# dlavado/scene-net

Measured on AMD Instinct MI355X. Metric: voxel-tiles/sec (point cloud -> 64^3 occupancy -> 16-GENEO bank conv -> head), higher is better.
Workload: dtype i8; 1 GPU; C2: 32 tiles/GPU x 100000 points (fp64 xyz, UTM-scale), 64^3 voxel grid, 16 GENEO kernels 9^3 (cy 6, cone 5, neg 5); conv on the int8 matrix cores: binary occupancy x 24-bit fixed-point weights (3 int8 digits), exact int32 accumulation, fp32 head; tiles_per_gpu=32, points_per_tile=100000, geneo_kernels=16, parallelism=tile-sharded x1, no collectives

## Files before the change

include/scenenet_hip.h:

```cpp
#ifndef SCENENET_HIP_H
#define SCENENET_HIP_H

#include <stddef.h>
#include <stdint.h>

#ifdef __cplusplus
extern "C" {
#endif

typedef void* sn_stream_t;

typedef enum {
    SN_OK = 0,
    SN_ERR_INVALID_ARG = -1,
    SN_ERR_UNSUPPORTED = -2,
    SN_ERR_LAUNCH = -3,
    SN_ERR_NO_DEVICE = -4,
    SN_ERR_DEVICE_STATUS = -5
} sn_status;

typedef enum { SN_F32 = 0, SN_F64 = 1, SN_U8 = 2, SN_OCC8 = 3, SN_BF16 = 4, SN_I32 = 5 } sn_dtype;

typedef enum {
    SN_GENEO_CY = 0, SN_GENEO_CONE = 1, SN_GENEO_NEG = 2,
// ... 38 lines not shown
                 void* act, void* out, int out_dtype, sn_stream_t stream);

int sn_conv_bank_plan(int x_dtype, int B, int Z, int X, int Y, int G, int kz, int kx, int ky, int32_t* plan8);

#define SN_CONV_PREP_BYTES 16384
int sn_conv_bank_prep(const float* bank, int G, int kz, int kx, int ky, void* prep, sn_stream_t stream);
int sn_conv_bank_prepared(const void* x, int x_dtype, const float* bank, const float* lambdas, void* prep,
                          int B, int Z, int X, int Y, int G, int kz, int kx, int ky,
                          void* act, void* out, int out_dtype, sn_stream_t stream);
int sn_conv_bank_prepared_served(const void* x, int x_dtype, const float* bank, const float* lambdas, void* prep,
                                 int B, int Z, int X, int Y, int G, int kz, int kx, int ky,
                                 void* act, void* out, int out_dtype, sn_stream_t stream);
int sn_conv_prep_verdict_offset(void);
int sn_conv_i8_spin_timeouts(unsigned long long* count);
int sn_conv_i8z_round_counts(unsigned long long* counts2);
int sn_voxel_onepass_giveups(unsigned long long* count);

int sn_launch_timing_events(void* start_event, void* stop_event);

int sn_conv_fused(const void* x, int x_dtype, const float* bank, const float* lambdas, int B, int Z, int X, int Y,
                  int G, int kz, int kx, int ky, void* out, int out_dtype, sn_stream_t stream);
int sn_conv_fused_v(const void* x, int x_dtype, const float* bank, const float* lambdas, int B, int Z, int X, int Y, int G,
                    int kz, int kx, int ky, void* out, int out_dtype, int32_t* verdict, int assume_served,
                    sn_stream_t stream);
size_t sn_conv_fused_prep_bytes(int kz, int kx, int ky);
int sn_conv_fused_prep(const float* bank, const float* lambdas, int G, int kz, int kx, int ky, void* blob,
                       sn_stream_t stream);
int sn_conv_fused_prepared(const void* x, int x_dtype, const float* bank, const float* lambdas, const void* blob, int B,
                           int Z, int X, int Y, int G, int kz, int kx, int ky, void* out, int out_dtype, int assume_served,
                           sn_stream_t stream);
// ... 406 lines not shown
```

scene-net_amd/_hip.py:

```python
from __future__ import annotations

import contextlib
import ctypes
import functools
import os
from ctypes import c_char_p, c_int, c_void_p
from typing import NamedTuple, Optional, Sequence, Tuple

import torch

_HERE = os.path.dirname(os.path.abspath(__file__))
LIB_PATH = os.environ.get("SN_HIP_LIB") or os.path.join(_HERE, "lib", "libscenenet_hip.so")

SN_F32, SN_F64, SN_U8, SN_OCC8, SN_BF16, SN_I32 = 0, 1, 2, 3, 4, 5
SN_GENEO_CY, SN_GENEO_CONE, SN_GENEO_NEG = 0, 1, 2
SN_GENEO_CY_V1, SN_GENEO_CONE_V1, SN_GENEO_NEG_V1 = 3, 4, 5
SN_P_RADIUS, SN_P_SIGMA, SN_P_APEX, SN_P_CONE_RADIUS, SN_P_CONE_INC, SN_P_NEG_FACTOR = 0, 1, 2, 3, 4, 5
SN_NPARAM = 8

_P, _I = c_void_p, c_int
SYMBOLS = {
    "sn_version": (c_int, []),
    "sn_prepare_device": (c_int, []),
    "sn_device_status": (c_int, [_P, _P]),
# ... 2 lines not shown
    "sn_device_count": (c_int, []),
    "sn_conv_i8_path_counts": (c_int, [_P]),
    "sn_set_option": (c_int, [c_char_p, _I]),
    "sn_get_option": (c_int, [c_char_p]),
    "sn_geneo_bank": (c_int, [_P, _P, _I, _I, _I, _I, _P, _P, _P]),
    "sn_effective_lambdas": (c_int, [_P, _P, _I, _I, _P, _P]),
    "sn_conv_bank": (c_int, [_P, _I, _P, _P, _I, _I, _I, _I, _I, _I, _I, _I, _P, _P, _I, _P]),
    "sn_conv_bank_plan": (c_int, [_I, _I, _I, _I, _I, _I, _I, _I, _I, _P]),
    "sn_geneo_bank_prep": (c_int, [_P, _P, _I, _I, _I, _I, _P, _P, _P, _P, _I, _P, _P, _P]),
    "sn_conv_bank_prep": (c_int, [_P, _I, _I, _I, _I, _P, _P]),
    "sn_conv_bank_prepared": (c_int, [_P, _I, _P, _P, _P, _I, _I, _I, _I, _I, _I, _I, _I, _P, _P, _I, _P]),
    "sn_conv_bank_prepared_served": (c_int, [_P, _I, _P, _P, _P, _I, _I, _I, _I, _I, _I, _I, _I, _P, _P, _I, _P]),
    "sn_conv_prep_verdict_offset": (c_int, []),
    "sn_conv_i8_spin_timeouts": (c_int, [_P]),
    "sn_conv_i8z_round_counts": (c_int, [_P]),
    "sn_voxel_onepass_giveups": (c_int, [_P]),
    "sn_launch_timing_events": (c_int, [_P, _P]),
    "sn_conv_fused": (c_int, [_P, _I, _P, _P, _I, _I, _I, _I, _I, _I, _I, _I, _P, _I, _P]),
    "sn_conv_fused_supported": (c_int, [_I, _I, _I, _I, _I, _I, _I]),
    "sn_forward_auto": (c_int, [_P, _I, _P, _P, _I, _I, _I, _I, _I, _I, _I, _I, _P, _P, _P, _I, _P]),
    "sn_voxel_bbox": (c_int, [_P, _P, _I, _P, _P]),
    "sn_voxel_desc": (c_int, [_P, _I, _I, _I, _I, _I, _P, _P]),
    "sn_voxel_desc_from_bounds": (c_int, [_P, _I, _I, _I, _I, _P, _P]),
    "sn_voxel_desc_sized": (c_int, [_P, _I, _P, _I, _I, _I, _P, _P, _P, _P]),
    "sn_voxel_finalize_sized": (c_int, [_P, _P, _I, _I, _I, _I, _P, _P, _P, _P, _P, _P, _P]),
    "sn_voxel_scatter": (c_int, [_P, _P, _P, _I, _P, _I, _I, _I, _P, _P, _P, _I, _P, _P]),
    "sn_voxel_finalize": (c_int, [_P, _P, _I, _I, _I, _I, _P, _P, _P, _P, _P, _P]),
    "sn_voxel_occupancy": (c_int, [_P, _P, _P, _I, _P, _I, _I, _I, _P, _I, _P, _P, _P, _I, _P, _P, _P, _P, _P]),
    "sn_voxel_occupancy_fused": (c_int, [_P, _P, _P, _I, _I, _I, _I, _I, _P, _I, _P, _P, _P, _P, _P, _P, _I, _P, _P, _P, _P,
                                         _P]),
# ... 209 lines not shown
    return int(buf[0]), int(buf[1]), int(buf[2])


def conv_i8_spin_timeouts() -> int:
    buf = (ctypes.c_ulonglong * 1)()
    _check(load().sn_conv_i8_spin_timeouts(ctypes.cast(buf, ctypes.c_void_p)), "sn_conv_i8_spin_timeouts")
    return int(buf[0])


def conv_i8z_round_counts() -> Tuple[int, int]:
    buf = (ctypes.c_ulonglong * 2)()
    _check(load().sn_conv_i8z_round_counts(ctypes.cast(buf, ctypes.c_void_p)), "sn_conv_i8z_round_counts")
    return int(buf[0]), int(buf[1])


def voxel_onepass_giveups() -> int:
    buf = (ctypes.c_ulonglong * 1)()
    _check(load().sn_voxel_onepass_giveups(ctypes.cast(buf, ctypes.c_void_p)), "sn_voxel_onepass_giveups")
    return int(buf[0])


def launch_timing_events(start: "torch.cuda.Event", stop: "torch.cuda.Event") -> None:
    a, b = int(start.cuda_event), int(stop.cuda_event)
    if not a or not b:
        raise HipLibraryError("launch_timing_events: record each event once first (torch creates the handle lazily)")
    _check_plain(load().sn_launch_timing_events(ctypes.c_void_p(a), ctypes.c_void_p(b)), "sn_launch_timing_events")


def _ptr(t: Optional[torch.Tensor], dtype: Optional[torch.dtype] = None, name: str = "tensor") -> Optional[int]:
    if t is None:
# ... 1728 lines not shown
```

scene-net_amd/csrc/cabi.hip:

```cpp
#include "common.h"
#include <climits>
#include <cstdlib>
#include <cstring>

#include <atomic>
#include <mutex>
#include <unordered_map>

namespace sn {
char* error_buffer() {
    static thread_local char buf[512] = {0};
    return buf;
}
namespace {
struct Option {
    const char* name;
    const char* env;
    int on;
    int def, lo, hi;
    bool is_switch;
    std::atomic<int> value{env ? -1 : def};
};
Option g_options[] = {
    {"conv_skip_empty_tiles",  nullptr,                 0,  0,       0,  1,       true},
    {"conv_i8_tolerance_ppb",  nullptr,                 0,  90000,   0,  INT_MAX, false},
    {"conv_i8_fold",           "SN_CONV_I8_NOFOLD",     0,  1,       0,  1,       true},
    {"conv_i8_legacy",         "SN_CONV_I8_LEGACY",     1,  0,       0,  1,       true},
    {"conv_i8_no_stage",       "SN_CONV_I8_NO_STAGE",   1,  0,       0,  1,       true},
    {"conv_i8z_variant",       nullptr,                 0,  2,       0,  2,       false},
    {"conv_no_i8",             "SN_CONV_NO_I8",         1,  0,       0,  1,       true},
    {"conv_double_buffer",     "SN_CONV_DOUBLE_BUFFER", 1,  0,       0,  1,       true},
    {"conv_lin_no24",          "SN_CONV_LIN_NO24",      1,  0,       0,  1,       true},
    {"voxel_onepass",          nullptr,                 0,  1,       0,  1,       true},
    {"voxel_onepass_spin",     nullptr,                 0,  64,      0,  INT_MAX, false},
    {"corr_dense",             "SN_CORR_DENSE",         1,  0,       0,  1,       true},
    {"corr_sparse_tile_bytes", nullptr,                 0,  0,       0,  2048,    false},
    {"conv_i8z_inject_fault",  nullptr,                 0,  0,       0,  1,       true},
    {"conv_i8z_segments",      nullptr,                 0,  0,       0,  4,       false},
    {"conv_i8z_dense",         nullptr,                 0,  0,       0,  1,       true},
};
static_assert(sizeof(g_options) / sizeof(g_options[0]) == kOptCount, "one entry per sn::Opt");
}

int option(Opt which) {
    Option& o = g_options[which];
    int v = o.value.load(std::memory_order_relaxed);
    if (v < 0) {
        const char* e = getenv(o.env);
        int expected = -1;
        o.value.compare_exchange_strong(expected, (e && e[0] == '1') ? o.on : o.def, std::memory_order_relaxed);
        v = o.value.load(std::memory_order_relaxed);
    }
    return v;
// ... 194 lines not shown
```

scene-net_amd/csrc/common.h:

```cpp
#pragma once
#include <hip/hip_runtime.h>
#include <cstdarg>
#include <cstdio>
#include <cstdlib>
#include "scenenet_hip.h"

namespace sn {

char* error_buffer();

inline int fail(int code, const char* fmt, ...) {
    va_list ap;
    va_start(ap, fmt);
    vsnprintf(error_buffer(), 512, fmt, ap);
    va_end(ap);
    return code;
}

int sticky_check(const char* what);

inline int check_launch(const char* what) {
    hipError_t e = hipGetLastError();
    if (e != hipSuccess) return fail(SN_ERR_LAUNCH, "%s: %s", what, hipGetErrorString(e));
    return sticky_check(what);
// ... 5 lines not shown
    kOptConvSkipEmptyTiles,
    kOptConvI8TolerancePpb,
    kOptConvI8Fold,
    kOptConvI8Legacy,
    kOptConvI8NoStage,
    kOptConvI8zVariant,
    kOptConvNoI8,
    kOptConvDoubleBuffer,
    kOptConvLinNo24,
    kOptVoxelOnepass,
    kOptVoxelOnepassSpin,
    kOptCorrDense,
    kOptCorrSparseTileBytes,
    kOptConvI8zInjectFault,
    kOptConvI8zSegments,
    kOptConvI8zDense,
    kOptCount
};
int option(Opt which);
inline float conv_i8_tolerance() { return 1e-9f * (float)option(kOptConvI8TolerancePpb); }

hipError_t ensure_dynamic_lds(const void* kernel, int bytes);

constexpr int kGateDepth = 3;
struct Gate {
    const int32_t* ptr[kGateDepth];
    int want[kGateDepth];
    __device__ __forceinline__ bool pass() const {
#pragma unroll
        for (int i = 0; i < kGateDepth; ++i)
// ... 67 lines not shown
```

scene-net_amd/csrc/conv_i8s.hip:

```cpp
#include "common.h"
#include <hip/hip_ext.h>
#include <cstdlib>
#include <cstring>
#include <type_traits>
#include <vector>

namespace {

#include "conv_prep.h"
#include "conv_fp32.inc"

#include "conv_i8_common.inc"
#include "conv_i8s_kernel.inc"
#include "conv_i8f.inc"

size_t lds_bytes_fold(const Shape& s) {
    const size_t hdw = (size_t)s.ZP * s.XP * DW;
    const size_t ring = kNB * hdw * 4, alias = 2 * hdw * 4 + ((size_t)s.G * 729 + 1) * sizeof(float);
    return (size_t)kFoldSteps * 3 * 64 * 16 + 64 + 64 + 128 + 128 + 64 + sizeof(FoldPlan) +
           (ring > alias ? ring : alias) + 16;
}

void plan_fold(int XP, FoldPlan& p) {
    for (int qq = 0; qq < 4; ++qq) {
// ... 244 lines not shown
    }
    if (best_cost < 0) return 1;
    if (!z.dense && SN_I8Z_SKIP_NSEG > 0 && SN_I8Z_SKIP_NSEG <= max_seg &&
        (ncol * SN_I8Z_SKIP_NSEG + cus - 1) / cus <= kZMaxJobs) {
        best_seg = SN_I8Z_SKIP_NSEG;
        z.deal = 1;
        z.deal_shift = SN_I8Z_SKIP_SHIFT;
    } else if (!z.dense) {
        const int want = sn::option(sn::kOptConvI8zSegments);
        const int n = want >= 2 ? want : (want == 0 && !act && z.nxt >= 2 && Z >= 32 && best_seg == 1) ? 2 : 0;
        if (n >= 2 && n <= max_seg && (ncol * n + cus - 1) / cus <= kZMaxJobs) {
            best_seg = n;
            z.deal = 1;
            z.deal_shift = z.nxt / n > 1 ? z.nxt / n : 1;
            z.fill_dead = act ? 0 : 1;
        }
    }
    z.LZ = (Z + best_seg - 1) / best_seg;
    z.nseg = (Z + z.LZ - 1) / z.LZ;
    z.PL = z.LZ + 8;
    const long long njobs = ncol * z.nseg;
    if (njobs > 0x7fffffff) return 1;
    z.njobs = (int)njobs;
    const int grid = (int)(njobs < cus ? njobs : cus);
    const int per_wg = (z.njobs + grid - 1) / grid;
    if (per_wg > kZMaxJobs) return 1;
    if (!division_magic((unsigned)z.PL, (unsigned)(per_wg * z.PL + 64), z.pl_magic)) return 1;
    z.swizzle = (grid % 8 == 0) ? 1 : 0;
    const size_t lds = lds_bytes_zwalk();
    const size_t lds_4 = lds_bytes(s4), lds_f = fp32k::lds_bytes(cs, false);
    const size_t lds_fb = lds_4 > lds_f ? lds_4 : lds_f;
    if (lds > (size_t)kMaxLds || lds_fb > (size_t)kMaxLds) return 1;
    hipEvent_t t_start = nullptr, t_stop = nullptr;
    sn::take_timing_events(t_start, t_stop);
#define SN_LAUNCH_I8Z(OT, KH, KR, KW)                                                                            \
    do {                                                                                                         \
        auto kern = act ? conv_occ_i8z_kernel<OT, KH, KR, KW, true> : conv_occ_i8z_kernel<OT, KH, KR, KW, false>; \
        if (sn::ensure_dynamic_lds((const void*)kern, kMaxLds) != hipSuccess)                                    \
            return check_launch("sn_conv_bank_prepared(i8z: hipFuncSetAttribute)");                              \
        if (t_start || t_stop)               \
            hipExtLaunchKernelGGL(kern, dim3(grid), dim3(64 * KW), (uint32_t)lds, stream, t_start, t_stop, 0u, x, lambdas,  \
                                  (const uint8_t*)prep, z, (OT*)act, (OT*)out);                                   \
        else                                                                                                     \
            hipLaunchKernelGGL(kern, dim3(grid), dim3(64 * KW), lds, stream, x, lambdas, (const uint8_t*)prep, z,   \
// ... 98 lines not shown
                                            void* out, int out_dtype, sn_stream_t stream) {
    return conv_bank_prepared_impl(x, x_dtype, bank, lambdas, prep, B, Z, X, Y, G, kz, kx, ky, act, out, out_dtype, stream, 1);
}

extern "C" int sn_conv_prep_verdict_offset(void) { return kPrepRoute; }

extern "C" int sn_conv_i8_path_counts(unsigned long long* counts3) {
    if (!counts3) return sn::fail(SN_ERR_INVALID_ARG, "sn_conv_i8_path_counts: null pointer");
    unsigned long long h[4] = {0, 0, 0, 0};
    if (hipDeviceSynchronize() != hipSuccess || hipMemcpyFromSymbol(h, HIP_SYMBOL(g_fold_counts), sizeof(h)) != hipSuccess)
        return sn::check_launch("sn_conv_i8_path_counts");
    counts3[0] = h[0]; counts3[1] = h[1]; counts3[2] = h[2];
    return SN_OK;
}

extern "C" int sn_conv_i8z_round_counts(unsigned long long* counts2) {
    if (!counts2) return sn::fail(SN_ERR_INVALID_ARG, "sn_conv_i8z_round_counts: null pointer");
    unsigned long long h[2] = {0, 0};
    if (hipDeviceSynchronize() != hipSuccess || hipMemcpyFromSymbol(h, HIP_SYMBOL(g_zwalk_rounds), sizeof(h)) != hipSuccess)
        return sn::check_launch("sn_conv_i8z_round_counts");
    counts2[0] = h[0]; counts2[1] = h[1];
    return SN_OK;
}

extern "C" int sn_conv_i8_spin_timeouts(unsigned long long* count) {
    if (!count) return sn::fail(SN_ERR_INVALID_ARG, "sn_conv_i8_spin_timeouts: null pointer");
    unsigned long long h[4] = {0, 0, 0, 0};
    if (hipDeviceSynchronize() != hipSuccess || hipMemcpyFromSymbol(h, HIP_SYMBOL(g_fold_counts), sizeof(h)) != hipSuccess)
        return sn::check_launch("sn_conv_i8_spin_timeouts");
    *count = h[3];
// ... 11 lines not shown
```

scene-net_amd/csrc/conv_i8z.inc:

```

constexpr int kZTX = 8;
constexpr int kZRows = kZTX + 8;
constexpr int kZRing = 16;
#ifndef SN_I8Z_LAG
#define SN_I8Z_LAG 3
#endif
constexpr int kZLag = SN_I8Z_LAG;
constexpr int kZD = 8 + kZLag;
#ifndef SN_I8Z_DD
#define SN_I8Z_DD 4
#endif
constexpr int kZDD = SN_I8Z_DD;
constexpr int kZPre = kZD + kZDD;
constexpr int kZRawPlane = kZRows * DW * 4;
constexpr int kZYqRow = 256, kZYqPlane = kZRows * kZYqRow;
constexpr int kZYcRow = 64, kZYcPlane = kZRows * kZYcRow + 32;
constexpr int kZMaxJobs = 256;
#ifndef SN_I8Z_SKIP_NSEG
#define SN_I8Z_SKIP_NSEG 0
#endif
#ifndef SN_I8Z_SKIP_SHIFT
#define SN_I8Z_SKIP_SHIFT 0
#endif
#ifndef SN_I8Z_AHEAD
// ... 14 lines not shown
    int njobs;
    unsigned pl_magic;
    int swizzle;
    float tol;
    sn::Gate gate;
    int32_t* route;
    int served;
    int fill_dead;
    int32_t* sticky;
    int dbg;
    int dense;
    int deal, deal_shift;
};

__device__ unsigned long long g_zwalk_rounds[2] = {0ull, 0ull};

__device__ __forceinline__ int zjob_id(const ZShape& z, int wg, int k, int grid) {
    const int base = k * grid;
    if (z.swizzle && base + grid <= z.njobs) return base + (wg & 7) * (grid >> 3) + (wg >> 3);
    return base + wg;
}

constexpr int kPrepThreads = SN_BANK_THREADS;
__global__ __launch_bounds__(kPrepThreads) void conv_prep_kernel(const float* __restrict__ bank, int G,
                                                                 uint8_t* __restrict__ prep) {
    __shared__ __align__(16) float w[732 + kPrepScratchWords];
    const int g = blockIdx.x, tid = threadIdx.x;
    const bool valid = g < G;
    for (int i = tid; i < 729; i += kPrepThreads) w[i] = valid ? bank[(size_t)g * 729 + i] : 0.0f;
    prep_one_kernel(w, w + 732, valid, g, prep, tid, kPrepThreads);
// ... 189 lines not shown
    const int lane = tid & 63, wave = __builtin_amdgcn_readfirstlane(tid >> 6);
    uint4* Wd = reinterpret_cast<uint4*>(lds);
    int4* jobtab = reinterpret_cast<int4*>(Wd + kFoldSteps * 3 * 64);
    float* scale = reinterpret_cast<float*>(jobtab + kZMaxJobs);
    float* lamsc = scale + 16;
    float* lamhi = lamsc + 16;
    double* bnd = reinterpret_cast<double*>(lamhi + 32);
    int* cnt = reinterpret_cast<int*>(bnd + 16);
    int4* chk = reinterpret_cast<int4*>(cnt + 128);
    int4* ltab = chk + 64;
    int4* stab = ltab + 64;
    uint32_t* rowmask = reinterpret_cast<uint32_t*>(stab + 64);
    uint8_t* raw = reinterpret_cast<uint8_t*>(rowmask + 32);
    uint8_t* Yc = raw + kZRing * kZRawPlane;
    uint8_t* Yq = Yc + kZRing * kZYcPlane;
    int* const ticket_ctr = cnt + 96;

#ifdef SN_CONV_TIMING
    if (lane < 8 && wave < 8) g_i8s_w[(blockIdx.x * 8 + wave) * 8 + lane] = 0;
#define SN_ZT(k, t0) do { if (lane == 0 && wave < 8) g_i8s_w[(blockIdx.x * 8 + wave) * 8 + (k)] += clock64() - (t0); } while (0)
#define SN_ZNOW() clock64()
#else
#define SN_ZT(k, t0) do { (void)(t0); } while (0)
#define SN_ZNOW() 0ull
#endif
    SN_ST(0);
    const size_t V = (size_t)zs.Z * zs.X * zs.Y;
    const int grid = (int)gridDim.x;
    const int dealt = (int)blockIdx.x < zs.njobs ? (zs.njobs - 1 - (int)blockIdx.x) / grid + 1 : 0;
    int my_jobs = dealt;
    int NPL = my_jobs * zs.PL;
    int nslots = NPL + kZD;
    const bool fill_dead = kLean && zs.fill_dead != 0;
    int* const live = reinterpret_cast<int*>(Yq);
    if (tid < 128) cnt[tid] = 0;
    if (tid >= 128 && tid < 192) {
        const int l = tid - 128, i = l & 15, role = l >> 4;
        int4 e = make_int4(0, 0, 0, 0);
        if (role == 0 && i <= 8) e = make_int4(i - kZD, 0, 1, 2);
        if (role == 1 && i <= 8) e = make_int4(i - kZRing + kZLag, 16, 2, kTShift);
        if (l == 32) e = make_int4(0, 32, 2 | 0x30, 0);
        if (l == 40) e = make_int4(kZDD - 16, 0, 4, 2);
        if (l == 48) e = make_int4(-kZRing, 16, 8, kTShift);
        chk[l] = e;
    }
    if (tid >= 192 && tid < 256) {
        const int l = tid - 192;
        ltab[l] = make_int4((l & 15) * 16, (l >> 4) * 256, 4 * (l & 15) + (l >> 4), (l >> 4) * 16);
    }
// ... 7 lines not shown
    if (tid < my_jobs) {
        int j = zjob_id(zs, (int)blockIdx.x, tid, grid);
        int xt, yt, sg;
        if (zs.deal) {
            const int ncol = zs.B * zs.nxt * zs.nyt;
            sg = j / ncol; j -= sg * ncol;
            xt = j % zs.nxt; j /= zs.nxt;
            yt = j % zs.nyt; j /= zs.nyt;
            xt = (xt + zs.deal_shift * sg) % zs.nxt;
        } else {
            xt = j % zs.nxt; j /= zs.nxt;
            yt = j % zs.nyt; j /= zs.nyt;
            sg = j % zs.nseg; j /= zs.nseg;
        }
        jobtab[tid] = make_int4(j, xt * kZTX, yt * TY, sg * zs.LZ);
    }
    if constexpr (kLean) {
        if (fill_dead)
            for (int i = tid; i < kZMaxJobs; i += kNT) live[i] = 0;
    }
    lds_barrier();

    struct JobRegs { int k, b, x0, y0, zs; };
    auto job_fetch = [&](JobRegs& jr, int k) -> bool {
        if (k == jr.k) return false;
        const int4 jb = jobtab[k];
        jr.b = __builtin_amdgcn_readfirstlane(jb.x); jr.x0 = __builtin_amdgcn_readfirstlane(jb.y);
        jr.y0 = __builtin_amdgcn_readfirstlane(jb.z); jr.zs = __builtin_amdgcn_readfirstlane(jb.w);
        jr.k = k;
        return true;
    };
    JobRegs jd{-1, 0, 0, 0, 0}, jr{-1, 0, 0, 0, 0};
    const uint8_t* xb = x;
    OT* ob = nullptr;

    auto dma_pass = [&](int u, int xr, int ln) {
        const int dl_row = (ln * 43) >> 8, dl_i = ln - dl_row * kRowPieces;
        const int k = (int)__umulhi((unsigned)u, zs.pl_magic), p = u - k * zs.PL;
        const bool new_job = job_fetch(jd, k);
        if constexpr (kLean) {
            if (new_job) xb = x + (size_t)jd.b * V;
        }
        const int gz = jd.zs - 4 + p;
        const int gx = jd.x0 - 4 + 4 * xr + dl_row, gy = jd.y0 - PYA + 16 * dl_i;
        const bool ok = (unsigned)gz < (unsigned)zs.Z && (unsigned)gx < (unsigned)zs.X && (unsigned)gy < (unsigned)zs.Y;
        uint8_t* const dst = raw + (u & 15) * kZRawPlane + xr * (4 * DW * 4);
        const uint32_t lds_uni = __builtin_amdgcn_readfirstlane((uint32_t)(uintptr_t)(__attribute__((address_space(3))) uint8_t*)dst);
        const uint8_t* const tile = kLean ? xb : x + (size_t)jd.b * V;
        const uint8_t* src = ok ? tile + (unsigned)((gz * zs.X + gx) * zs.Y + gy) : prep + kPrepZero;
        if (ln < 4 * kRowPieces) {
            uint32_t m0_saved;
            asm volatile("; @zw:dma\n\ts_mov_b32 %0, m0\n\ts_mov_b32 m0, %1\n\ts_nop 0\n\tglobal_load_lds_dwordx4 %2, off\n\t"
                         "s_mov_b32 m0, %0"
                         : "=&s"(m0_saved) : "s"(lds_uni), "v"(src) : "memory");
        }
    };
// ... 22 lines not shown
            const int4 jb = jobtab[k];
            for (int r = wave; r < zs.LZ * kZTX; r += kW) {
                const int gz = jb.w + (r >> 3), gx = jb.y + (r & 7), gy = jb.z + lane;
                if (gz >= zs.Z || gx >= zs.X || gy >= zs.Y) continue;
                const size_t off = ((size_t)gz * zs.X + gx) * zs.Y + gy;
                if (out) out[(size_t)jb.x * V + off] = nan;
                if (act)
                    for (int g = 0; g < zs.G; ++g) act[((size_t)jb.x * zs.Gtot + zs.g0 + g) * V + off] = nan;
            }
        }
    };

    int npre = NPL < kZPre ? NPL : kZPre;
    if (!fill_dead)
        for (int p = wave; p < 4 * npre; p += kW) dma_pass(p >> 2, p & 3, lane);
    auto region_or2 = [&](int k0, uint32_t& a0, uint32_t& a1) {
        static_assert(kNT % 128 == 0, "a thread's (row, piece) is the same for every plane it takes");
        constexpr int kStep = kNT / 128, kBatch = 8;
        const int pc = tid & 7, row = (tid >> 3) & 15;
        const bool two = k0 + 1 < dealt;
        const int4 j0 = jobtab[k0], j1 = jobtab[two ? k0 + 1 : k0];
        const int gx0 = j0.y - 4 + row, gy0 = j0.z - PYA + 16 * pc, gx1 = j1.y - 4 + row, gy1 = j1.z - PYA + 16 * pc;
        const bool in0 = pc < kRowPieces && (unsigned)gx0 < (unsigned)zs.X && (unsigned)gy0 < (unsigned)zs.Y;
        const bool in1 = two && pc < kRowPieces && (unsigned)gx1 < (unsigned)zs.X && (unsigned)gy1 < (unsigned)zs.Y;
        const int plane = zs.X * zs.Y;
        const uint8_t* const t0 = x + (size_t)j0.x * V + (unsigned)(in0 ? gx0 * zs.Y + gy0 : 0);
        const uint8_t* const t1 = x + (size_t)j1.x * V + (unsigned)(in1 ? gx1 * zs.Y + gy1 : 0);
        const uint32_t kx = pc == kRowPieces - 1 ? ~0u : pc == 0 ? 0u : ~0u, kyz = (pc == 0 || pc == kRowPieces - 1) ? 0u : ~0u,
                       kw = pc == 0 ? ~0u : pc == kRowPieces - 1 ? 0u : ~0u;
#pragma unroll 1
        for (int pl0 = tid >> 7; pl0 < zs.PL; pl0 += kStep * kBatch) {
            uint4 v0[kBatch], v1[kBatch];
            bool ok0[kBatch], ok1[kBatch];
#pragma unroll
            for (int u = 0; u < kBatch; ++u) {
                const int pl = pl0 + u * kStep, gz0 = j0.w - 4 + pl, gz1 = j1.w - 4 + pl;
                ok0[u] = in0 && pl < zs.PL && (unsigned)gz0 < (unsigned)zs.Z;
                ok1[u] = in1 && pl < zs.PL && (unsigned)gz1 < (unsigned)zs.Z;
                v0[u] = *reinterpret_cast<const uint4*>(t0 + (unsigned)(ok0[u] ? gz0 * plane : 0));
                v1[u] = *reinterpret_cast<const uint4*>(t1 + (unsigned)(ok1[u] ? gz1 * plane : 0));
            }
#pragma unroll
            for (int u = 0; u < kBatch; ++u) {
                const uint32_t w0 = (v0[u].x & kx) | ((v0[u].y | v0[u].z) & kyz) | (v0[u].w & kw);
                const uint32_t w1 = (v1[u].x & kx) | ((v1[u].y | v1[u].z) & kyz) | (v1[u].w & kw);
                a0 |= ok0[u] ? w0 : 0u;
                a1 |= ok1[u] ? w1 : 0u;
            }
        }
    };
    auto region_report = [&](int k, uint32_t a) {
        if (__builtin_amdgcn_ballot_w64(a != 0u) != 0ull && lane == 0) live[k] = 1;
    };
    if constexpr (kLean) {
        if (fill_dead) {
#pragma unroll 1
            for (int k = 0; k < dealt; k += 2) {
                uint32_t a0 = 0u, a1 = 0u;
                region_or2(k, a0, a1);
                region_report(k, a0);
                region_report(k + 1, a1);
            }
        }
    }
    {
        const uint4* src = reinterpret_cast<const uint4*>(prep + kPrepWd);
        for (int i = tid; i < kFoldSteps * 3 * 64; i += kNT) Wd[i] = src[i];
        if (tid < 16) {
            scale[tid] = reinterpret_cast<const float*>(prep + kPrepScale)[tid];
            bnd[tid] = reinterpret_cast<const double*>(prep + kPrepBnd)[tid];
            lamhi[16 + tid] = (lambdas && tid < zs.G) ? lambdas[tid] : 0.0f;
            if (tid < zs.G && reinterpret_cast<const int*>(prep + kPrepSym)[tid] == 0) cnt[97] = 1;
        }
        if (tid >= 64 && tid < 128) cnt[32 + tid - 64] = (((tid - 64) & 15) < npre && !((zs.dbg & 1) && tid == 64)) ? 1 : 0;
    }
    lds_barrier();
    bool early = false;
    if constexpr (kLean) {
        if (fill_dead && dealt > 0 && zs.PL >= kZPre && __builtin_amdgcn_readfirstlane(live[0]) != 0) {
            early = true;
            for (int p = wave; p < 4 * npre; p += kW) dma_pass(p >> 2, p & 3, lane);
        }
    }
    {
        const bool asym = cnt[97] != 0;
        const bool exceeded = !asym && bound_exceeded<OT>(zs, bnd, lamhi + 16, act, out);
        if (blockIdx.x == 0 && tid == 0) {
            if (zs.route) *zs.route = asym ? 2 : exceeded ? 1 : 0;
            atomicAdd(&g_fold_counts[asym ? 1 : exceeded ? 2 : 0], 1ull);
        }
        if (asym || exceeded) {
            asm volatile("s_waitcnt vmcnt(0)" ::: "memory");
            if (zs.served) {
                poison_jobs();
// ... 6 lines not shown
        bool fin = true;
        if (tid < 16) {
            const float sc = scale[tid];
            const float ls = (out && tid < zs.G) ? lamhi[16 + tid] * sc : 0.0f;
            const float lh = 65536.0f * ls;
            lamsc[tid] = ls;
            lamhi[tid] = lh;
            auto finite = [](float v) { return (__float_as_uint(v) & 0x7f800000u) != 0x7f800000u; };
            fin = finite(sc) && !(__float_as_uint(sc) >> 31) && finite(ls) && finite(lh);
        }
        const bool all_fin = __builtin_amdgcn_ballot_w64(!fin) == 0ull;
        if (lane == 0) cnt[99] = (all_fin && !zs.dense) ? 1 : 0;
        if constexpr (kLean) {
            if (fill_dead) {
                const bool may_skip = all_fin && !zs.dense;
                int4* const old = reinterpret_cast<int4*>(Yq + kZMaxJobs * 4);
                int nlive = 0;
#pragma unroll 1
                for (int k0 = 0; k0 < dealt; k0 += 64) {
                    const int k = k0 + lane;
                    const bool lv = k < dealt && (!may_skip || live[k] != 0);
                    if (k < dealt) {
                        old[k] = jobtab[k];
                        live[k] = lv ? 1 : 0;
                    }
                    nlive += __builtin_popcountll(__builtin_amdgcn_ballot_w64(lv));
                }
                int at_live = 0, at_dead = nlive;
#pragma unroll 1
                for (int k0 = 0; k0 < dealt; k0 += 64) {
                    const int k = k0 + lane;
                    const bool in = k < dealt, lv = in && live[k] != 0;
                    const unsigned long long ml = __builtin_amdgcn_ballot_w64(lv), md = __builtin_amdgcn_ballot_w64(in && !lv);
                    const unsigned long long m = lv ? ml : md;
                    const int rank = (int)__builtin_amdgcn_mbcnt_hi((uint32_t)(m >> 32), __builtin_amdgcn_mbcnt_lo((uint32_t)m, 0u));
                    if (in) jobtab[(lv ? at_live : at_dead) + rank] = old[k];
                    at_live += __builtin_popcountll(ml);
                    at_dead += __builtin_popcountll(md);
                }
                if (lane == 0) cnt[103] = nlive;
            }
        }
    }
    asm volatile("s_waitcnt vmcnt(0)" ::: "memory");
    __syncthreads();
    if (my_jobs == 0) return;
    const bool can_skip = __builtin_amdgcn_readfirstlane(cnt[99]) != 0;
    int n_run = 0, n_skip = 0;
    if constexpr (kLean) {
        if (fill_dead) {
            my_jobs = __builtin_amdgcn_readfirstlane(cnt[103]);
            NPL = my_jobs * zs.PL;
            nslots = NPL + kZD;
            if (!early) {
                npre = NPL < kZPre ? NPL : kZPre;
                for (int p = wave; p < 4 * npre; p += kW) dma_pass(p >> 2, p & 3, lane);
                if (tid >= 64 && tid < 128) cnt[32 + tid - 64] = (((tid - 64) & 15) < npre && !((zs.dbg & 1) && tid == 64)) ? 1 : 0;
            }
            int dead_rounds = 0;
#pragma unroll 1
            for (int k = my_jobs; k < dealt; ++k) {
                const int4 jb = jobtab[k];
                const int nz = zs.Z - jb.w < zs.LZ ? zs.Z - jb.w : zs.LZ;
                const int nx = zs.X - jb.y < kZTX ? zs.X - jb.y : kZTX;
                const int ny4 = (zs.Y - jb.z < TY ? zs.Y - jb.z : TY) >> 2;
                dead_rounds += nz * ((nx + kH - 1) / kH);
                if (!out) continue;
                OT* const tile = out + (size_t)jb.x * V;
#pragma unroll 1
                for (int i = tid; i < nz * (kZTX * 16); i += kNT) {
                    const int yq = i & 15, xr = (i >> 4) & (kZTX - 1), pz = i >> 7;
                    if (yq >= ny4 || xr >= nx) continue;
                    OT* const o = tile + (unsigned)(((jb.w + pz) * zs.X + jb.y + xr) * zs.Y + jb.z + 4 * yq);
                    float t[4] = {0.0f, 0.0f, 0.0f, 0.0f};
                    asm volatile("" : "+v"(t[0]), "+v"(t[1]), "+v"(t[2]), "+v"(t[3]));
                    if (zs.head & 1) {
                        if constexpr (sizeof(OT) == 4) {
                            const float4 v = *reinterpret_cast<const float4*>(o);
                            t[0] += v.x; t[1] += v.y; t[2] += v.z; t[3] += v.w;
                        } else {
                            const double2 v = reinterpret_cast<const double2*>(o)[0], w = reinterpret_cast<const double2*>(o)[1];
                            t[0] += (float)v.x; t[1] += (float)v.y; t[2] += (float)w.x; t[3] += (float)w.y;
                        }
                    }
                    if (zs.head & 2) {
#pragma unroll
                        for (int e = 0; e < 4; ++e) t[e] = relu_tanh(t[e]);
// ... 14 lines not shown
            if (!early) {
                asm volatile("s_waitcnt vmcnt(0)" ::: "memory");
                __syncthreads();
            }
        }
    }
    SN_ST(4);

    bool healthy = true;
    const int ntickets = kTPS * nslots;
    auto claim = [&]() -> int {
        int t = 0;
        if (lane == 0) t = __hip_atomic_fetch_add(ticket_ctr, 1, __ATOMIC_RELAXED, __HIP_MEMORY_SCOPE_WORKGROUP);
        return __builtin_amdgcn_readfirstlane(t);
    };
    int pend = -1;
    auto signal_passes = [&](int first) { lds_add_lane0<1>(&cnt[first], 1, lane); };

    int next = claim();
    for (int t = next; t < ntickets; t = next) {
        const unsigned long long tz0 = SN_ZNOW();
        next = claim();
        int ln = lane;
        asm volatile("" : "+v"(ln));
        const int s = t >> kTShift, tk = t & (kTPS - 1);
        int4 LT, ST;
        if constexpr (!kLean) {
            LT = ltab[ln];
            ST = *reinterpret_cast<const int4*>(reinterpret_cast<const uint8_t*>(stab) + ((s - kZD) & 15) * 64 + (ln & 0x30));
        }
        const bool pass_ticket = kTPS <= 4 || (tk & 1) == 0;
        const int xr0 = kTPS == 8 ? tk >> 1 : tk;
        const int sd = s + kZDD;
        const bool has_dma = pass_ticket && s >= kZD && sd < NPL;
        const bool has_fold = pass_ticket && s < NPL;
        const int sigma = s - kZD;
        int kr = 0, o = 0;
        bool has_round = false;
        if (sigma >= 0) {
            kr = (int)__umulhi((unsigned)sigma, zs.pl_magic);
            o = sigma - kr * zs.PL;
            has_round = o < zs.LZ;
        }
        if (pend >= 0) {
            asm volatile("; @zw:wait1\n\ts_waitcnt vmcnt(0)" ::: "memory");
            signal_passes(pend);
            pend = -1;
        }
        SN_ZT(0, tz0);
        const unsigned long long tz1 = SN_ZNOW();
        int midx;
        {
            const int4 role = chk[ln];
            const int have = (has_round ? 1 : 0) | (has_fold ? 2 : 0) | (has_dma ? 4 : 0) | 8;
            const int v = s + role.x;
            const int idx = ((v & 15) | role.y) + (role.z & (xr0 * 16));
            const int expect = ((role.z & have) && v >= 0) ? (((v >> 4) + 1) << role.w) : 0;
// ... 27 lines not shown
        if (has_dma) {
            dma_pass(sd, xr0, ln);
            pend = 32 + xr0 * 16 + (sd & 15);
        }
        if (has_fold) {
            fold_pass(s, xr0, ln);
            lds_add_lane0<2>(&cnt[s & 15], 1, lane);
        }
        SN_ZT(2, tz2);
        if (!has_round) {
            asm volatile("; @zw:wait3\n\ts_waitcnt lgkmcnt(0)" ::: "memory");
            lds_add_lane0<3>(&cnt[16 + (s & 15)], 1, lane);
            continue;
        }
        const unsigned long long tz3 = SN_ZNOW();
        const bool new_job = job_fetch(jr, kr);
        if constexpr (kLean) {
            if (new_job && out) ob = out + (size_t)jr.b * V;
        }
        const int gz = jr.zs + o;
        const int lx = kH * kR * tk;
        int rows_left = 0, nvalid = 0;
        if (gz >= zs.Z || jr.x0 + lx >= zs.X) {
            asm volatile("; @zw:wait3\n\ts_waitcnt lgkmcnt(0)" ::: "memory");
            lds_add_lane0<3>(&cnt[16 + (s & 15)], 1, lane);
            continue;
        }
        if constexpr (kLean) {
            rows_left = zs.X - (jr.x0 + lx);
            nvalid = rows_left >= kH * kR ? kR : (rows_left + kH - 1) / kH;
        }
        if (kLean && can_skip) {
            const uint32_t ub = zwindow_mask<kH * kR>(kH * kR == 2 ? (tk & 1) * 2 : (tk & 3), kH * kR == 2 ? tk >> 1 : tk >> 2);
// ... 251 lines not shown
        }
        SN_ZT(6, tz0);
    }
    SN_ST(5);
    if (pend >= 0) {
        asm volatile("; @zw:wait1\n\ts_waitcnt vmcnt(0)" ::: "memory");
        signal_passes(pend);
    }
    if (lane == 0) {
        const uint32_t a = (uint32_t)(uintptr_t)(__attribute__((address_space(3))) int*)(cnt + 100);
        asm volatile("ds_add_u32 %0, %1\n\tds_add_u32 %0, %2 offset:4" ::"v"(a), "v"(n_run), "v"(n_skip) : "memory");
        if (atomicInc(reinterpret_cast<unsigned*>(cnt + 102), 0xffffffffu) == (unsigned)kW - 1u) {
            const volatile __attribute__((address_space(3))) int* tot = (__attribute__((address_space(3))) int*)cnt;
            atomicAdd(&g_zwalk_rounds[0], (unsigned long long)(unsigned)tot[100]);
            atomicAdd(&g_zwalk_rounds[1], (unsigned long long)(unsigned)tot[101]);
        }
    }
    asm volatile("s_waitcnt vmcnt(0)" ::: "memory");
    if (reinterpret_cast<const volatile __attribute__((address_space(3))) int*>((__attribute__((address_space(3))) int*)cnt)[98] != 0) {
        __syncthreads();
        poison_jobs();
        if (!healthy && lane == 0) atomicAdd(&g_fold_counts[3], 1ull);
    }
}

template <typename OT>
__global__ __launch_bounds__(kThreads) void conv_i8_fallback_kernel(const uint8_t* __restrict__ x,
                                                                    const float* __restrict__ bank,
                                                                    const float* __restrict__ lambdas,
                                                                    const int32_t* __restrict__ route, Shape s4,
                                                                    fp32k::ConvShape cs, OT* __restrict__ act,
                                                                    OT* __restrict__ out) {
    if (!cs.gate.pass()) return;
    const int verdict = *route;
    if (verdict <= 0) return;
    bool to_fp32 = verdict == 1;
    if (verdict == 2) {
        to_fp32 = conv_occ_i8s_body<OT, 10, 6, 1>(x, bank, lambdas, s4, act, out);
        if (to_fp32) __syncthreads();
    }
    if (to_fp32) fp32k::conv_bank_body<uint8_t, OT, false>(x, bank, lambdas, cs, act, out);
}

size_t lds_bytes_zwalk() {
    return (size_t)kFoldSteps * 3 * 64 * 16 + (size_t)kZMaxJobs * 16 + 64 * 4 + 128 + 128 * 4 + 64 * 16 + 2 * 64 * 16 +
           32 * 4 + (size_t)kZRing * (kZRawPlane + kZYcPlane + kZYqPlane) + 16;
}

bool division_magic(unsigned d, unsigned umax, unsigned& magic) {
    magic = (unsigned)((((unsigned long long)1 << 32) / d) + 1ull);
    for (unsigned u = 0; u <= umax; ++u)
        if ((unsigned)(((unsigned long long)u * magic) >> 32) != u / d) return false;
    return true;
}
```

Baseline: 302,900 tiles/s.

## Trim z-walk conv to occupied z-plane runs instead of whole live jobs

```diff
diff --git a/include/scenenet_hip.h b/include/scenenet_hip.h
--- a/include/scenenet_hip.h
+++ b/include/scenenet_hip.h
@@ -76,6 +76,7 @@
 int sn_conv_prep_verdict_offset(void);
 int sn_conv_i8_spin_timeouts(unsigned long long* count);
 int sn_conv_i8z_round_counts(unsigned long long* counts2);
+int sn_conv_i8z_planes_streamed(unsigned long long* count);
 int sn_voxel_onepass_giveups(unsigned long long* count);
 
 int sn_launch_timing_events(void* start_event, void* stop_event);
diff --git a/scene-net_amd/_hip.py b/scene-net_amd/_hip.py
--- a/scene-net_amd/_hip.py
+++ b/scene-net_amd/_hip.py
@@ -40,6 +40,7 @@
     "sn_conv_prep_verdict_offset": (c_int, []),
     "sn_conv_i8_spin_timeouts": (c_int, [_P]),
     "sn_conv_i8z_round_counts": (c_int, [_P]),
+    "sn_conv_i8z_planes_streamed": (c_int, [_P]),
     "sn_voxel_onepass_giveups": (c_int, [_P]),
     "sn_launch_timing_events": (c_int, [_P, _P]),
     "sn_conv_fused": (c_int, [_P, _I, _P, _P, _I, _I, _I, _I, _I, _I, _I, _I, _P, _I, _P]),
@@ -279,6 +280,12 @@
     return int(buf[0]), int(buf[1])
 
 
+def conv_i8z_planes_streamed() -> int:
+    buf = (ctypes.c_ulonglong * 1)()
+    _check(load().sn_conv_i8z_planes_streamed(ctypes.cast(buf, ctypes.c_void_p)), "sn_conv_i8z_planes_streamed")
+    return int(buf[0])
+
+
 def voxel_onepass_giveups() -> int:
     buf = (ctypes.c_ulonglong * 1)()
     _check(load().sn_voxel_onepass_giveups(ctypes.cast(buf, ctypes.c_void_p)), "sn_voxel_onepass_giveups")
diff --git a/scene-net_amd/csrc/cabi.hip b/scene-net_amd/csrc/cabi.hip
--- a/scene-net_amd/csrc/cabi.hip
+++ b/scene-net_amd/csrc/cabi.hip
@@ -37,6 +37,7 @@
     {"corr_sparse_tile_bytes", nullptr,                 0,  0,       0,  2048,    false},
     {"conv_i8z_inject_fault",  nullptr,                 0,  0,       0,  1,       true},
     {"conv_i8z_segments",      nullptr,                 0,  0,       0,  4,       false},
+    {"conv_i8z_trim",          "SN_CONV_I8Z_TRIM",      1,  0,       0,  1,       true},
     {"conv_i8z_dense",         nullptr,                 0,  0,       0,  1,       true},
 };
 static_assert(sizeof(g_options) / sizeof(g_options[0]) == kOptCount, "one entry per sn::Opt");
diff --git a/scene-net_amd/csrc/common.h b/scene-net_amd/csrc/common.h
--- a/scene-net_amd/csrc/common.h
+++ b/scene-net_amd/csrc/common.h
@@ -43,6 +43,7 @@
     kOptCorrSparseTileBytes,
     kOptConvI8zInjectFault,
     kOptConvI8zSegments,
+    kOptConvI8zTrim,
     kOptConvI8zDense,
     kOptCount
 };
diff --git a/scene-net_amd/csrc/conv_i8s.hip b/scene-net_amd/csrc/conv_i8s.hip
--- a/scene-net_amd/csrc/conv_i8s.hip
+++ b/scene-net_amd/csrc/conv_i8s.hip
@@ -282,6 +282,7 @@
             z.deal = 1;
             z.deal_shift = z.nxt / n > 1 ? z.nxt / n : 1;
             z.fill_dead = act ? 0 : 1;
+            if (z.fill_dead && sn::option(sn::kOptConvI8zTrim) && (Z + n - 1) / n <= 64) z.fill_dead |= 2;
         }
     }
     z.LZ = (Z + best_seg - 1) / best_seg;
@@ -295,7 +296,7 @@
     if (per_wg > kZMaxJobs) return 1;
     if (!division_magic((unsigned)z.PL, (unsigned)(per_wg * z.PL + 64), z.pl_magic)) return 1;
     z.swizzle = (grid % 8 == 0) ? 1 : 0;
-    const size_t lds = lds_bytes_zwalk();
+    const size_t lds = lds_bytes_zwalk(!act);
     const size_t lds_4 = lds_bytes(s4), lds_f = fp32k::lds_bytes(cs, false);
     const size_t lds_fb = lds_4 > lds_f ? lds_4 : lds_f;
     if (lds > (size_t)kMaxLds || lds_fb > (size_t)kMaxLds) return 1;
@@ -424,6 +425,16 @@
     return SN_OK;
 }
 
+extern "C" int sn_conv_i8z_planes_streamed(unsigned long long* count) {
+    if (!count) return sn::fail(SN_ERR_INVALID_ARG, "sn_conv_i8z_planes_streamed: null pointer");
+    unsigned long long h[kZCountSlots][16];
+    if (hipDeviceSynchronize() != hipSuccess || hipMemcpyFromSymbol(h, HIP_SYMBOL(g_zwalk_planes), sizeof(h)) != hipSuccess)
+        return sn::check_launch("sn_conv_i8z_planes_streamed");
+    *count = 0ull;
+    for (int i = 0; i < kZCountSlots; ++i) *count += h[i][0];
+    return SN_OK;
+}
+
 extern "C" int sn_conv_i8z_round_counts(unsigned long long* counts2) {
     if (!counts2) return sn::fail(SN_ERR_INVALID_ARG, "sn_conv_i8z_round_counts: null pointer");
     unsigned long long h[2] = {0, 0};
diff --git a/scene-net_amd/csrc/conv_i8z.inc b/scene-net_amd/csrc/conv_i8z.inc
--- a/scene-net_amd/csrc/conv_i8z.inc
+++ b/scene-net_amd/csrc/conv_i8z.inc
@@ -52,6 +52,30 @@
 };
 
 __device__ unsigned long long g_zwalk_rounds[2] = {0ull, 0ull};
+constexpr int kZCountSlots = 64;
+__device__ unsigned long long g_zwalk_planes[kZCountSlots][16] = {};
+
+__device__ __forceinline__ unsigned long long zrun_close(unsigned long long needed) {
+    unsigned long long runs = 0ull, rest = needed;
+    while (rest) {
+        const int a = __builtin_ctzll(rest);
+        int e = a;
+        while (true) {
+            const unsigned long long x = ~(rest >> e);
+            e += x ? __builtin_ctzll(x) : 64;
+            if (e >= 64) { e = 64; break; }
+            const unsigned long long tail = rest >> e;
+            if (!tail) break;
+            const int gap = __builtin_ctzll(tail);
+            if (gap > 8) break;
+            e += gap;
+        }
+        const unsigned long long m = (e >= 64 ? ~0ull : (1ull << e) - 1ull) & ~((1ull << a) - 1ull);
+        runs |= m;
+        rest &= ~m;
+    }
+    return runs;
+}
 
 __device__ __forceinline__ int zjob_id(const ZShape& z, int wg, int k, int grid) {
     const int base = k * grid;
@@ -271,6 +295,10 @@
     uint8_t* raw = reinterpret_cast<uint8_t*>(rowmask + 32);
     uint8_t* Yc = raw + kZRing * kZRawPlane;
     uint8_t* Yq = Yc + kZRing * kZYcPlane;
+    int4* etab = reinterpret_cast<int4*>(Yq + kZRing * kZYqPlane);
+    int2* elen = reinterpret_cast<int2*>(Wd + kFoldSteps * 3 * 64);
+    if constexpr (kLean) jobtab = etab + kZMaxJobs;
+    unsigned long long* runm = reinterpret_cast<unsigned long long*>(etab + 2 * kZMaxJobs);
     int* const ticket_ctr = cnt + 96;
 
 #ifdef SN_CONV_TIMING
@@ -288,8 +316,9 @@
     int my_jobs = dealt;
     int NPL = my_jobs * zs.PL;
     int nslots = NPL + kZD;
-    const bool fill_dead = kLean && zs.fill_dead != 0;
-    int* const live = reinterpret_cast<int*>(Yq);
+    const bool fill_dead = kLean && (zs.fill_dead & 1) != 0;
+    const bool trim = fill_dead && (zs.fill_dead & 2) != 0;
+    uint32_t* const pbits = reinterpret_cast<uint32_t*>(Yq);
     if (tid < 128) cnt[tid] = 0;
     if (tid >= 128 && tid < 192) {
         const int l = tid - 128, i = l & 15, role = l >> 4;
@@ -327,14 +356,18 @@
             sg = j % zs.nseg; j /= zs.nseg;
         }
         jobtab[tid] = make_int4(j, xt * kZTX, yt * TY, sg * zs.LZ);
+        if constexpr (kLean) {
+            etab[tid] = make_int4(j, xt * kZTX, yt * TY, sg * zs.LZ);
+            elen[tid] = make_int2(tid * zs.PL, tid * zs.PL + zs.PL);
+        }
     }
     if constexpr (kLean) {
         if (fill_dead)
-            for (int i = tid; i < kZMaxJobs; i += kNT) live[i] = 0;
+            for (int i = tid; i < 4 * dealt; i += kNT) pbits[i] = 0u;
     }
     lds_barrier();
 
-    struct JobRegs { int k, b, x0, y0, zs; };
+    struct JobRegs { int k, b, x0, y0, zs, u0, end; };
     auto job_fetch = [&](JobRegs& jr, int k) -> bool {
         if (k == jr.k) return false;
         const int4 jb = jobtab[k];
@@ -343,16 +376,42 @@
         jr.k = k;
         return true;
     };
-    JobRegs jd{-1, 0, 0, 0, 0}, jr{-1, 0, 0, 0, 0};
+    auto entry_seek = [&](JobRegs& jr, int u) -> bool {
+        if (u < jr.end) return false;
+        do {
+            ++jr.k;
+            constexpr int kElenOff = kFoldSteps * 3 * 64 * 16;
+            const uint32_t elen0 = (uint32_t)(uintptr_t)(__attribute__((address_space(3))) int2*)elen - (uint32_t)kElenOff;
+            int2 e;
+            asm volatile("ds_read_b64 %0, %1 offset:%c2\n\ts_waitcnt lgkmcnt(0)"
+                         : "=v"(e) : "v"(elen0 + (uint32_t)jr.k * 8u), "i"(kElenOff) : "memory");
+            jr.u0 = __builtin_amdgcn_readfirstlane(e.x);
+            jr.end = __builtin_amdgcn_readfirstlane(e.y);
+        } while (u >= jr.end && jr.k < kZMaxJobs - 1);
+        return true;
+    };
+    auto entry_load = [&](JobRegs& jr) {
+        const int4 jb = etab[jr.k];
+        jr.b = __builtin_amdgcn_readfirstlane(jb.x); jr.x0 = __builtin_amdgcn_readfirstlane(jb.y);
+        jr.y0 = __builtin_amdgcn_readfirstlane(jb.z); jr.zs = __builtin_amdgcn_readfirstlane(jb.w);
+    };
+    JobRegs jd{-1, 0, 0, 0, 0, 0, 0}, jr{-1, 0, 0, 0, 0, 0, 0};
     const uint8_t* xb = x;
     OT* ob = nullptr;
 
     auto dma_pass = [&](int u, int xr, int ln) {
         const int dl_row = (ln * 43) >> 8, dl_i = ln - dl_row * kRowPieces;
-        const int k = (int)__umulhi((unsigned)u, zs.pl_magic), p = u - k * zs.PL;
-        const bool new_job = job_fetch(jd, k);
+        int p;
         if constexpr (kLean) {
-            if (new_job) xb = x + (size_t)jd.b * V;
+            if (entry_seek(jd, u)) {
+                entry_load(jd);
+                xb = x + (size_t)jd.b * V;
+            }
+            p = u - jd.u0;
+        } else {
+            const int k = (int)__umulhi((unsigned)u, zs.pl_magic);
+            p = u - k * zs.PL;
+            job_fetch(jd, k);
         }
         const int gz = jd.zs - 4 + p;
         const int gx = jd.x0 - 4 + 4 * xr + dl_row, gy = jd.y0 - PYA + 16 * dl_i;
@@ -405,7 +464,8 @@
     int npre = NPL < kZPre ? NPL : kZPre;
     if (!fill_dead)
         for (int p = wave; p < 4 * npre; p += kW) dma_pass(p >> 2, p & 3, lane);
-    auto region_or2 = [&](int k0, uint32_t& a0, uint32_t& a1) {
+    struct PlaneBits { unsigned long long lo; uint32_t hi; };
+    auto region_or2 = [&](int k0, PlaneBits& a0, PlaneBits& a1) {
         static_assert(kNT % 128 == 0, "a thread's (row, piece) is the same for every plane it takes");
         constexpr int kStep = kNT / 128, kBatch = 8;
         const int pc = tid & 7, row = (tid >> 3) & 15;
@@ -419,8 +479,9 @@
         const uint8_t* const t1 = x + (size_t)j1.x * V + (unsigned)(in1 ? gx1 * zs.Y + gy1 : 0);
         const uint32_t kx = pc == kRowPieces - 1 ? ~0u : pc == 0 ? 0u : ~0u, kyz = (pc == 0 || pc == kRowPieces - 1) ? 0u : ~0u,
                        kw = pc == 0 ? ~0u : pc == kRowPieces - 1 ? 0u : ~0u;
+        uint32_t any0 = 0u, any1 = 0u;
 #pragma unroll 1
-        for (int pl0 = tid >> 7; pl0 < zs.PL; pl0 += kStep * kBatch) {
+        for (int pl0 = wave >> 1; pl0 < zs.PL; pl0 += kStep * kBatch) {
             uint4 v0[kBatch], v1[kBatch];
             bool ok0[kBatch], ok1[kBatch];
 #pragma unroll
@@ -435,19 +496,39 @@
             for (int u = 0; u < kBatch; ++u) {
                 const uint32_t w0 = (v0[u].x & kx) | ((v0[u].y | v0[u].z) & kyz) | (v0[u].w & kw);
                 const uint32_t w1 = (v1[u].x & kx) | ((v1[u].y | v1[u].z) & kyz) | (v1[u].w & kw);
-                a0 |= ok0[u] ? w0 : 0u;
-                a1 |= ok1[u] ? w1 : 0u;
-            }
+                if (!trim) {
+                    any0 |= ok0[u] ? w0 : 0u;
+                    any1 |= ok1[u] ? w1 : 0u;
+                    continue;
+                }
+                const int bit = pl0 + u * kStep;
+                const unsigned long long blo = bit < 64 ? 1ull << bit : 0ull;
+                const uint32_t bhi = bit < 64 ? 0u : 1u << ((bit - 64) & 31);
+                if (__builtin_amdgcn_ballot_w64(ok0[u] && w0 != 0u) != 0ull) { a0.lo |= blo; a0.hi |= bhi; }
+                if (__builtin_amdgcn_ballot_w64(ok1[u] && w1 != 0u) != 0ull) { a1.lo |= blo; a1.hi |= bhi; }
+            }
+        }
+        if (!trim) {
+            if (__builtin_amdgcn_ballot_w64(any0 != 0u) != 0ull) a0.lo = 1ull;
+            if (__builtin_amdgcn_ballot_w64(any1 != 0u) != 0ull) a1.lo = 1ull;
         }
     };
-    auto region_report = [&](int k, uint32_t a) {
-        if (__builtin_amdgcn_ballot_w64(a != 0u) != 0ull && lane == 0) live[k] = 1;
+    auto region_report = [&](int k, const PlaneBits& a) {
+        if (lane == 0 && k < dealt) {
+            if (!trim) {
+                if (a.lo) pbits[4 * k] = 1u;
+                return;
+            }
+            if ((uint32_t)a.lo) atomicOr(&pbits[4 * k], (uint32_t)a.lo);
+            if ((uint32_t)(a.lo >> 32)) atomicOr(&pbits[4 * k + 1], (uint32_t)(a.lo >> 32));
+            if (a.hi) atomicOr(&pbits[4 * k + 2], a.hi);
+        }
     };
     if constexpr (kLean) {
         if (fill_dead) {
 #pragma unroll 1
             for (int k = 0; k < dealt; k += 2) {
-                uint32_t a0 = 0u, a1 = 0u;
+                PlaneBits a0{0ull, 0u}, a1{0ull, 0u};
                 region_or2(k, a0, a1);
                 region_report(k, a0);
                 region_report(k + 1, a1);
@@ -468,7 +549,21 @@
     lds_barrier();
     bool early = false;
     if constexpr (kLean) {
-        if (fill_dead && dealt > 0 && zs.PL >= kZPre && __builtin_amdgcn_readfirstlane(live[0]) != 0) {
+        bool first_live = false;
+        if (fill_dead && dealt > 0 && zs.PL >= kZPre) {
+            const uint32_t b0 = __builtin_amdgcn_readfirstlane(pbits[0]), b1 = __builtin_amdgcn_readfirstlane(pbits[1]),
+                           b2 = __builtin_amdgcn_readfirstlane(pbits[2]);
+            if (!trim) {
+                first_live = (b0 | b1 | b2) != 0u;
+            } else {
+                uint32_t n = b0;
+#pragma unroll
+                for (int d = 1; d <= 8; ++d) n |= b0 >> d;
+                const int zs0 = __builtin_amdgcn_readfirstlane(jobtab[0].w);
+                first_live = (n & 0x7fu) == 0x7fu && zs.Z - zs0 >= 7 && zs.LZ >= 7;
+            }
+        }
+        if (first_live) {
             early = true;
             for (int p = wave; p < 4 * npre; p += kW) dma_pass(p >> 2, p & 3, lane);
         }
@@ -505,31 +600,102 @@
         if constexpr (kLean) {
             if (fill_dead) {
                 const bool may_skip = all_fin && !zs.dense;
-                int4* const old = reinterpret_cast<int4*>(Yq + kZMaxJobs * 4);
-                int nlive = 0;
+                const unsigned long long whole = ~0ull;
+                if (!trim) {
+                    int nlive = 0;
+#pragma unroll 1
+                    for (int k0 = 0; k0 < dealt; k0 += 64) {
+                        const int k = k0 + lane;
+                        const bool lv = k < dealt && (!may_skip || pbits[4 * k] != 0u);
+                        const unsigned long long ml = __builtin_amdgcn_ballot_w64(lv);
+                        const int e = nlive + (int)__builtin_amdgcn_mbcnt_hi((uint32_t)(ml >> 32), __builtin_amdgcn_mbcnt_lo((uint32_t)ml, 0u));
+                        if (k < dealt) runm[k] = lv ? whole : 0ull;
+                        if (lv) {
+                            etab[e] = jobtab[k];
+                            elen[e] = make_int2(e * zs.PL, e * zs.PL + zs.PL);
+                        }
+                        nlive += __builtin_popcountll(ml);
+                    }
+                    if (lane == 0) {
+                        cnt[103] = nlive;
+                        cnt[104] = nlive * zs.PL;
+                    }
+                } else {
+                int total = 0;
 #pragma unroll 1
                 for (int k0 = 0; k0 < dealt; k0 += 64) {
                     const int k = k0 + lane;
-                    const bool lv = k < dealt && (!may_skip || live[k] != 0);
+                    unsigned long long R = 0ull;
                     if (k < dealt) {
-                        old[k] = jobtab[k];
-                        live[k] = lv ? 1 : 0;
-                    }
-                    nlive += __builtin_popcountll(__builtin_amdgcn_ballot_w64(lv));
-                }
-                int at_live = 0, at_dead = nlive;
+                        const uint4 pb = *reinterpret_cast<const uint4*>(pbits + 4 * k);
+                        const unsigned long long lo = (unsigned long long)pb.x | ((unsigned long long)pb.y << 32);
+                        if (!may_skip) {
+                            R = whole;
+                        } else {
+                            unsigned long long n = lo;
+#pragma unroll
+                            for (int d = 1; d <= 8; ++d) n |= (lo >> d) | ((unsigned long long)pb.z << (64 - d));
+                            const int zs0 = jobtab[k].w;
+                            const int nz = zs.Z - zs0 < zs.LZ ? zs.Z - zs0 : zs.LZ;
+                            if (nz < 64) n &= (1ull << nz) - 1ull;
+                            R = zrun_close(n);
+                        }
+                        runm[k] = R;
+                    }
+                    if (dealt * 7 > kZMaxJobs) {
+                        int c = R == whole ? 1 : __builtin_popcountll(R & ~(R << 1));
+#pragma unroll
+                        for (int d = 32; d >= 1; d >>= 1) c += __shfl_xor(c, d);
+                        total += c;
+                    }
+                }
+                const bool all_whole = total > kZMaxJobs;
+                int e_base = 0, u_base = 0;
 #pragma unroll 1
                 for (int k0 = 0; k0 < dealt; k0 += 64) {
                     const int k = k0 + lane;
-                    const bool in = k < dealt, lv = in && live[k] != 0;
-                    const unsigned long long ml = __builtin_amdgcn_ballot_w64(lv), md = __builtin_amdgcn_ballot_w64(in && !lv);
-                    const unsigned long long m = lv ? ml : md;
-                    const int rank = (int)__builtin_amdgcn_mbcnt_hi((uint32_t)(m >> 32), __builtin_amdgcn_mbcnt_lo((uint32_t)m, 0u));
-                    if (in) jobtab[(lv ? at_live : at_dead) + rank] = old[k];
-                    at_live += __builtin_popcountll(ml);
-                    at_dead += __builtin_popcountll(md);
-                }
-                if (lane == 0) cnt[103] = nlive;
+                    unsigned long long R = k < dealt ? runm[k] : 0ull;
+                    if (all_whole && R != 0ull) {
+                        R = whole;
+                        runm[k] = R;
+                    }
+                    const int c = R == whole ? 1 : __builtin_popcountll(R & ~(R << 1));
+                    const int pl = R == whole ? zs.PL : __builtin_popcountll(R) + 8 * c;
+                    const int nact = dealt - k0 < 64 ? dealt - k0 : 64;
+                    int ec = c, up = pl;
+#pragma unroll 1
+                    for (int d = 1; d < nact; d <<= 1) {
+                        const int te = __shfl_up(ec, d), tu = __shfl_up(up, d);
+                        if (lane >= d) { ec += te; up += tu; }
+                    }
+                    int e = e_base + ec - c, u0 = u_base + up - pl;
+                    if (R != 0ull) {
+                        const int4 jb = jobtab[k];
+                        if (R == whole) {
+                            etab[e] = jb;
+                            elen[e] = make_int2(u0, u0 + zs.PL);
+                        } else {
+                            unsigned long long rest = R;
+                            while (rest) {
+                                const int a = __builtin_ctzll(rest);
+                                const unsigned long long x = ~(rest >> a);
+                                const int len = x ? __builtin_ctzll(x) : 64;
+                                etab[e] = make_int4(jb.x, jb.y, jb.z, jb.w + a);
+                                elen[e] = make_int2(u0, u0 + len + 8);
+                                ++e;
+                                u0 += len + 8;
+                                rest &= a + len >= 64 ? 0ull : ~0ull << (a + len);
+                            }
+                        }
+                    }
+                    e_base += __shfl(ec, nact - 1);
+                    u_base += __shfl(up, nact - 1);
+                }
+                if (lane == 0) {
+                    cnt[103] = e_base;
+                    cnt[104] = u_base;
+                }
+                }
             }
         }
     }
@@ -541,8 +707,9 @@
     if constexpr (kLean) {
         if (fill_dead) {
             my_jobs = __builtin_amdgcn_readfirstlane(cnt[103]);
-            NPL = my_jobs * zs.PL;
+            NPL = __builtin_amdgcn_readfirstlane(cnt[104]);
             nslots = NPL + kZD;
+            jd.k = -1; jd.u0 = 0; jd.end = 0;
             if (!early) {
                 npre = NPL < kZPre ? NPL : kZPre;
                 for (int p = wave; p < 4 * npre; p += kW) dma_pass(p >> 2, p & 3, lane);
@@ -550,18 +717,22 @@
             }
             int dead_rounds = 0;
 #pragma unroll 1
-            for (int k = my_jobs; k < dealt; ++k) {
+            for (int k = 0; k < dealt; ++k) {
+                const unsigned long long R = runm[k];
+                const uint32_t Rlo = __builtin_amdgcn_readfirstlane((uint32_t)R), Rhi = __builtin_amdgcn_readfirstlane((uint32_t)(R >> 32));
+                if ((Rlo & Rhi) == ~0u) continue;
+                const unsigned long long runs = (unsigned long long)Rlo | ((unsigned long long)Rhi << 32);
                 const int4 jb = jobtab[k];
                 const int nz = zs.Z - jb.w < zs.LZ ? zs.Z - jb.w : zs.LZ;
                 const int nx = zs.X - jb.y < kZTX ? zs.X - jb.y : kZTX;
                 const int ny4 = (zs.Y - jb.z < TY ? zs.Y - jb.z : TY) >> 2;
-                dead_rounds += nz * ((nx + kH - 1) / kH);
+                dead_rounds += (nz - __builtin_popcountll(runs)) * ((nx + kH - 1) / kH);
                 if (!out) continue;
                 OT* const tile = out + (size_t)jb.x * V;
 #pragma unroll 1
                 for (int i = tid; i < nz * (kZTX * 16); i += kNT) {
                     const int yq = i & 15, xr = (i >> 4) & (kZTX - 1), pz = i >> 7;
-                    if (yq >= ny4 || xr >= nx) continue;
+                    if (yq >= ny4 || xr >= nx || ((runs >> (pz & 63)) & 1ull)) continue;
                     OT* const o = tile + (unsigned)(((jb.w + pz) * zs.X + jb.y + xr) * zs.Y + jb.z + 4 * yq);
                     float t[4] = {0.0f, 0.0f, 0.0f, 0.0f};
                     asm volatile("" : "+v"(t[0]), "+v"(t[1]), "+v"(t[2]), "+v"(t[3]));
@@ -606,6 +777,7 @@
         if (lane == 0) t = __hip_atomic_fetch_add(ticket_ctr, 1, __ATOMIC_RELAXED, __HIP_MEMORY_SCOPE_WORKGROUP);
         return __builtin_amdgcn_readfirstlane(t);
     };
+    bool jr_new = false;
     int pend = -1;
     auto signal_passes = [&](int first) { lds_add_lane0<1>(&cnt[first], 1, lane); };
 
@@ -630,9 +802,15 @@
         int kr = 0, o = 0;
         bool has_round = false;
         if (sigma >= 0) {
-            kr = (int)__umulhi((unsigned)sigma, zs.pl_magic);
-            o = sigma - kr * zs.PL;
-            has_round = o < zs.LZ;
+            if constexpr (kLean) {
+                jr_new = entry_seek(jr, sigma) || jr_new;
+                o = sigma - jr.u0;
+                has_round = sigma + 8 < jr.end;
+            } else {
+                kr = (int)__umulhi((unsigned)sigma, zs.pl_magic);
+                o = sigma - kr * zs.PL;
+                has_round = o < zs.LZ;
+            }
         }
         if (pend >= 0) {
             asm volatile("; @zw:wait1\n\ts_waitcnt vmcnt(0)" ::: "memory");
@@ -690,9 +868,14 @@
             continue;
         }
         const unsigned long long tz3 = SN_ZNOW();
-        const bool new_job = job_fetch(jr, kr);
         if constexpr (kLean) {
-            if (new_job && out) ob = out + (size_t)jr.b * V;
+            if (jr_new) {
+                entry_load(jr);
+                if (out) ob = out + (size_t)jr.b * V;
+                jr_new = false;
+            }
+        } else {
+            job_fetch(jr, kr);
         }
         const int gz = jr.zs + o;
         const int lx = kH * kR * tk;
@@ -974,6 +1157,8 @@
             const volatile __attribute__((address_space(3))) int* tot = (__attribute__((address_space(3))) int*)cnt;
             atomicAdd(&g_zwalk_rounds[0], (unsigned long long)(unsigned)tot[100]);
             atomicAdd(&g_zwalk_rounds[1], (unsigned long long)(unsigned)tot[101]);
+            if constexpr (kLean)
+                atomicAdd(&g_zwalk_planes[blockIdx.x & (kZCountSlots - 1)][0], (unsigned long long)(unsigned)NPL);
         }
     }
     asm volatile("s_waitcnt vmcnt(0)" ::: "memory");
@@ -1002,9 +1187,9 @@
     if (to_fp32) fp32k::conv_bank_body<uint8_t, OT, false>(x, bank, lambdas, cs, act, out);
 }
 
-size_t lds_bytes_zwalk() {
+size_t lds_bytes_zwalk(bool head_only) {
     return (size_t)kFoldSteps * 3 * 64 * 16 + (size_t)kZMaxJobs * 16 + 64 * 4 + 128 + 128 * 4 + 64 * 16 + 2 * 64 * 16 +
-           32 * 4 + (size_t)kZRing * (kZRawPlane + kZYcPlane + kZYqPlane) + 16;
+           32 * 4 + (size_t)kZRing * (kZRawPlane + kZYcPlane + kZYqPlane) + (head_only ? (size_t)kZMaxJobs * (16 + 16 + 8) : 0) + 16;
 }
 
 bool division_magic(unsigned d, unsigned umax, unsigned& magic) {
```

Result: no change. 301,400 tiles/s (-0.5%).
